# Rinoahu/SwiftOrtho

Measured on AMD Instinct MI355X. Metric: M query-aa/s scanned all-vs-all, higher is better.
Workload: dtype u8/int16/int32 (5-bit packed residues, packed 16-bit score-only DP, int32 traced DP); 1 GPU; BASELINE config 3: 100000 synthetic proteins x 300 aa self-search, seed 11111011111, aa9, -M 120000000, -c 50000 (2 chunks), -e 1e-5, -v 500; query_aa=30007201, rows=1618760

## Files before the change

swiftortho_amd/csrc/host.h:

```cpp
#pragma once
#include "common.h"
#include "kernels.h"
#include "seedhash.h"
#include "../../include/sohit.h"

#include <algorithm>
#include <array>
#include <atomic>
#include <chrono>
#include <cmath>
#include <cstring>
#include <functional>
#include <map>
#include <malloc.h>
#include <memory>
#include <mutex>
#include <thread>
#include <unordered_map>
#include <sys/stat.h>

inline double wall() { return std::chrono::duration<double>(std::chrono::steady_clock::now().time_since_epoch()).count(); }

extern double (*volatile p_pow)(double, double);
extern double (*volatile p_log)(double);
// ... 64 lines not shown
    std::string header(i64 x) const { return data.substr(hd_beg[x], hd_len[x]); }
    std::string ident(i64 x) const {
        std::string h = header(x);
        return h.substr(0, h.find(' '));
    }
    u32 len(i64 x) const { return off[x + 1] - off[x]; }
};


struct ChunkIndex {
    u64 s2 = 0;
    i64 seq_lo = 0, seq_hi = 0;
    u32 p_lo = 0, p_hi = 0;
    u32 E = 0;
    i64 threshold = 0;
    u32 maxslen = 0;
    DevBuf<u64> entries;
    DevBuf<u32> ub, ubeg, ucnt;
    u32 U = 0;
    DevBuf<u32> hkey;
    DevBuf<u64> hval;
    int hshift = 31;
    u32 hmask = 0;
    DevBuf<u64> dir;
    bool use_dir = false;
    DevBuf<u64> dkeys;
    int d_sh_subj = -1, d_sh_diag = -1;
    struct BandEnc {
        int ba = -1, bp = -1, k = -1;
        bool multi_ok = false;
        bool multi = false;
        u32 nband = 0;
        u32 C = 0;
        DevBuf<u32> dk32, gbase;
        DevBuf<u64> btab;
        std::vector<std::pair<u32, u32>> spans;
        u64 used = 0;
        bool stale = false;
        u64 ref_gen = 0;
        i64 seq_lo = -1, seq_hi = -1;
    };
    std::vector<std::unique_ptr<BandEnc>> encs;
    u64 enc_clock = 0;
    bool ordered = false;
    DevBuf<u32> row_of_slot;
    struct RangeTab {
        int ba = -1, bp = -1, k = -1, wb = -1;
// ... 39 lines not shown
    DevBuf<int> d_bittab;
    u8 smap[256];
    signed char b62c[SCLS_N * SCLS_N];
    static const int BITTAB_N = 1 << 16;
    SeqSet ref, qry;
    std::string ref_path;
    long long ref_fsize = -1, ref_mtime_ns = -1;
    bool ref_loaded = false, qry_loaded = false, index_built = false;
    u64 ref_gen = 0;
    struct BandPlan { i64 lo, hi; int bp; bool multi_ok; int k; u64 nband; };
    std::vector<BandPlan> band_plans;
    i64 r_lo = -1, r_hi = -1;
    std::vector<std::unique_ptr<ChunkIndex>> chunks;
    std::vector<std::unique_ptr<ChunkIndex>> spare_chunks;
    std::vector<std::string> masked;
    i64 masked_lo = 0;
    std::vector<std::vector<u32>> last_cands;
    std::vector<std::array<int64_t, 8>> last_p2;
    u64 qry_gen = 0;
    i64 last_q_lo = 0;
    so_counters cnt;
    DevBuf<u32> d_scan_tmp, d_tmp32a, d_tmp32b;
    DevBuf<u64> d_stats;
    DevBuf<u32> d_small;
    DevBuf<u32> ix_bkt, ix_bkt2, ix_flags, ix_ridx, ix_plan, ix_tk;
    DevBuf<u64> ix_ent, ix_tv;
    DevBuf<u8> d_pcls;
    DevBuf<u8> d_sort_tmp;
    hipEvent_t ev0 = nullptr, ev1 = nullptr;
    hipStream_t st_rows = nullptr;
    hipEvent_t ev_rows = nullptr, ev_rows_done = nullptr;
    hipEvent_t ev_part[EMIT_PARTS_MAX] = {nullptr};
    hipStream_t st_side = nullptr;
    hipEvent_t ev_side_go = nullptr, ev_korder = nullptr;
    hipStream_t st_ug = nullptr;
    hipEvent_t ev_ug_go = nullptr, ev_ug_done = nullptr;
    hipEvent_t ev_bnd_go = nullptr, ev_bnd_done = nullptr;
    bool rows_in_flight = false;
    bool count_tab_now = false;
    size_t max_hits_per_pass = (size_t)1 << 30;
    u32 max_batch = 131072;
    DevBuf<u8> d_segtab, d_symmap, d_upmap, d_segmask;
    bool seg_on_device = false;
    bool q_present[256];
    void* pinned = nullptr;
    size_t pinned_cap = 0;
// ... 418 lines not shown
```

swiftortho_amd/csrc/host_index.hip:

```cpp
#include "host.h"


i64 chunk_threshold(so_ctx* c, const u32* d_counts , u64 s1, u64 s2, u64 nn) {
    const double N = (double)(nn + 1);
    const double mu = (double)s1 / N;
    long double lm = (long double)mu;
    long double ss = (long double)s2 - 2.0L * lm * (long double)s1 + (long double)nn * lm * lm;
    if (ss < 0) ss = 0;
    long double T = lm + 2.0L * sqrtl(ss / (long double)N);
    long double fl = floorl(T);
    long double margin = ((long double)nn * 8e-16L + 1e-11L) * (T + 1.0L);
    const bool forced = tune().exact_threshold;
    if (!forced && T - fl > margin && (fl + 1.0L) - T > margin) return (i64)fl;
    std::vector<u32> counts((size_t)nn);
    if (nn) HIP_CHECK(hipMemcpyAsync(counts.data(), d_counts, (size_t)nn * sizeof(u32), hipMemcpyDeviceToHost, c->st));
    HIP_CHECK(hipStreamSynchronize(c->st));
    i64 Nn = 1;
    double m = 0.;
    for (u32 v : counts)
        if (v > 0) m += (double)v, Nn += 1;
    m /= (double)Nn;
    double sd = 0.;
    for (u32 v : counts)
        if (v > 0) sd += p_pow((double)v - m, 2);
// ... 95 lines not shown
            dlap("alloc entries / grouping scratch");
            ixsort_finish(c->ix_bkt.p, c->ix_ent.p, nslots, (u32)NC, c->ix_plan.p, c->ix_tk.p, c->ix_tv.p, c->ix_bkt2.p, ch->entries.p, c->st);
            dlap("pair grouping");
            c->ix_flags.ensure((size_t)E + 4), c->ix_ridx.ensure((size_t)E + 4);
            c->d_scan_tmp.ensure(scan_u32_temp_elems((size_t)E + 1) + 8);
            launch_run_heads(c->ix_bkt2.p, E, c->ix_flags.p, c->st);
            const u32 U = d2h_u32(c, scan_u32(c->ix_flags.p, c->ix_ridx.p, E, false, c->d_scan_tmp.p, c->st));
            ch->U = U;
            ch->ub.ensure((size_t)U + 4), ch->ubeg.ensure((size_t)U + 4), ch->ucnt.ensure((size_t)U + 4);
            launch_run_list(c->ix_bkt2.p, c->ix_flags.p, c->ix_ridx.p, E, U, ch->ub.p, ch->ubeg.p, ch->ucnt.p, c->st);
            dlap("run heads / list");
            launch_index_stats(ch->ucnt.p, U, c->d_stats.p, c->st);
            u64* stats = (u64*)small_host(c);
            u32* last_lo_h = (u32*)(stats + 4);
            HIP_CHECK(hipMemcpyAsync(stats, c->d_stats.p, 4 * sizeof(u64), hipMemcpyDeviceToHost, c->st));
            HIP_CHECK(hipMemcpyAsync(last_lo_h, ch->ubeg.p + (U - 1), sizeof(u32), hipMemcpyDeviceToHost, c->st));
            HIP_CHECK(hipStreamSynchronize(c->st));
            s2 = stats[1];
            const u32 last_lo = *last_lo_h;
            dlap("stats");
            if (ch->use_dir) {
                const size_t nd = (size_t)NC / 32 + 2;
                ch->dir.ensure(nd);
                HIP_CHECK(hipMemsetAsync(ch->dir.p, 0, nd * sizeof(u64), c->st));
                launch_dir_build(ch->ub.p, U, ch->dir.p, c->st);
            } else {
                u32 cap = 1024;
                int lg = 10;
                while (cap < 2 * U) cap <<= 1, ++lg;
                ch->hkey.ensure(cap), ch->hval.ensure(cap);
                ch->hshift = 32 - lg, ch->hmask = cap - 1;
                HIP_CHECK(hipMemsetAsync(ch->hkey.p, 0xFF, (size_t)cap * sizeof(u32), c->st));
                launch_htab_insert(ch->ub.p, ch->ubeg.p, U, ch->hkey.p, ch->hval.p, ch->hshift, ch->hmask, c->st);
            }
            launch_index_fixlast(ch->entries.p, last_lo, E, c->st);
        } else if (ch->use_dir) {
            const size_t nd = (size_t)NC / 32 + 2;
            ch->dir.ensure(nd);
            ch->ubeg.ensure(4);
            HIP_CHECK(hipMemsetAsync(ch->dir.p, 0, nd * sizeof(u64), c->st));
        } else {
            ch->hkey.ensure(1024), ch->hval.ensure(1024);
            ch->hshift = 22, ch->hmask = 1023;
            HIP_CHECK(hipMemsetAsync(ch->hkey.p, 0xFF, 1024 * sizeof(u32), c->st));
        }
        dlap("directory + fixlast");
        ch->threshold = chunk_threshold(c, ch->ucnt.p, (u64)E, s2, (u64)ch->U);
        ch->s2 = s2;
        HIP_CHECK(hipStreamSynchronize(c->st));
        c->cnt.index_entries += ch->E;
        c->chunks.push_back(std::move(ch));
    }
    c->spare_chunks.clear();
    c->cnt.n_chunks = (i64)c->chunks.size();
    c->index_built = true;
    c->cnt.index_ms += (wall() - t0) * 1e3;
}


bool host_window_bucket(const so_ctx* c, const u8* seq, u32 len, u32 pos, int a, int s, u32* bucket) {
    const int k = c->cfg.klen[s];
    if ((u64)pos + (u64)k > (u64)len) return false;
    const u32 care = c->cfg.care[s];
// ... 116 lines not shown
                    }
                    const int before = (int)std::count(seen.begin(), seen.end(), e);
                    if (before >= nt) {
                        bad = true;
                        return;
                    }
                    seen.push_back(e);
                    ent[i] = e | ((u64)tags[nt - 1 - before] << 24);
                }
            });
            if (bad) throw SoError("so_load_index: " + name + ".idx does not match the loaded reference under these seeds (a slot's window does not hash to its bucket)");
        }
        ch->entries.ensure((size_t)E + 4);
        ch->ub.ensure((size_t)U + 4), ch->ubeg.ensure((size_t)U + 4), ch->ucnt.ensure((size_t)U + 4);
        if (E) HIP_CHECK(hipMemcpyAsync(ch->entries.p, ent.data(), (size_t)E * sizeof(u64), hipMemcpyHostToDevice, c->st));
        if (U) {
            HIP_CHECK(hipMemcpyAsync(ch->ub.p, ub.data(), (size_t)U * sizeof(u32), hipMemcpyHostToDevice, c->st));
            HIP_CHECK(hipMemcpyAsync(ch->ucnt.p, ucnt.data(), (size_t)U * sizeof(u32), hipMemcpyHostToDevice, c->st));
        }
        HIP_CHECK(hipMemcpyAsync(ch->ubeg.p, ubeg.data(), ((size_t)U + 1) * sizeof(u32), hipMemcpyHostToDevice, c->st));
        if (ch->use_dir) {
            const size_t nd = (size_t)NC / 32 + 2;
            ch->dir.ensure(nd);
            HIP_CHECK(hipMemsetAsync(ch->dir.p, 0, nd * sizeof(u64), c->st));
            if (U) launch_dir_build(ch->ub.p, U, ch->dir.p, c->st);
        } else {
            u32 cap = 1024;
            int lg = 10;
            while (cap < 2 * U) cap <<= 1, ++lg;
            ch->hkey.ensure(cap), ch->hval.ensure(cap);
            ch->hshift = 32 - lg, ch->hmask = cap - 1;
            HIP_CHECK(hipMemsetAsync(ch->hkey.p, 0xFF, (size_t)cap * sizeof(u32), c->st));
            if (U) launch_htab_insert(ch->ub.p, ch->ubeg.p, U, ch->hkey.p, ch->hval.p, ch->hshift, ch->hmask, c->st);
        }
        HIP_CHECK(hipStreamSynchronize(c->st));
        c->cnt.index_entries += ch->E;
        c->chunks.push_back(std::move(ch));
    }
    c->cnt.n_chunks = (i64)c->chunks.size();
    c->index_built = true;
    c->cnt.index_ms += (wall() - t0) * 1e3;
}


void band_plan(so_ctx* c, ChunkIndex& ch, int bp, bool multi_ok, int* k_out, u64* nband_out) {
    for (const auto& pl : c->band_plans)
        if (pl.lo == ch.seq_lo && pl.hi == ch.seq_hi && pl.bp == bp && pl.multi_ok == multi_ok) {
            *k_out = pl.k, *nband_out = pl.nband;
// ... 147 lines not shown
```

swiftortho_amd/csrc/host_seed.hip:

```cpp
#include "host.h"

static void defer_long_class(so_ctx* c, Batch& b, u32 q_long) {
    b.korder_async = q_long < b.nq && b.cls_sorted && b.qcls[q_long] != b.qcls[0];
    if (!b.korder_async) return;
    b.q_defer = q_long;
    while (b.q_defer > 0 && b.qcls[b.q_defer - 1] == b.qcls[q_long]) --b.q_defer;
    HIP_CHECK(hipEventRecord(c->ev_side_go, c->st));
    HIP_CHECK(hipStreamWaitEvent(c->st_side, c->ev_side_go, 0));
}

void order_queries(so_ctx* c, Batch& b) {
    const u32 q_long = b.ksc_long;
    const size_t nres = b.h_off[b.nq];
    if (q_long < b.nq) b.gx.ensure(nres + 4), b.gL.ensure(nres + 4), b.gR.ensure(nres + 4);
    defer_long_class(c, b, q_long);
    launch_ksc_order(b.dev.d_scls.p, b.dev.d_off.p, b.nq, q_long, c->cfg.mink, c->d_b62c.p, b.gx.p, b.gL.p, b.gR.p, b.korder.p, c->st,
                     b.korder_async ? c->st_side : c->st);
    if (b.korder_async) HIP_CHECK(hipEventRecord(c->ev_korder, c->st_side));
    b.korder_ready = true;
}

void order_open_queries(so_ctx* c, Batch& b, const unsigned long long* qh) {
    u32 q_long = b.nq;
    for (u32 q = b.ksc_long; q < b.nq && q_long == b.nq; ++q)
// ... 153 lines not shown
    HIP_CHECK(hipMemcpyAsync(v, c->d_small.p + SM_STASH0, 2 * sizeof(u32), hipMemcpyDeviceToHost, c->st));
    HIP_CHECK(hipStreamSynchronize(c->st));
    a = v[0], b = v[1];
}

void ensure_sort_tmp(so_ctx* c, size_t bytes) { c->d_sort_tmp.ensure(bytes + 256); }

const unsigned long long* chunk_qhits(so_ctx* c, Batch& b, int ci) {
    ChunkIndex& ch = *c->chunks[ci];
    const int AS = c->cfg.A * c->cfg.S;
    const u32 Ppad = b.dev.Ppad, NC = (u32)c->nc;
    if (b.bnd_ci == ci) {
        HIP_CHECK(hipStreamWaitEvent(c->st, c->ev_bnd_done, 0));
        std::swap(b.sbeg.p, b.sbeg2.p), std::swap(b.sbeg.cap, b.sbeg2.cap);
        std::swap(b.scnt.p, b.scnt2.p), std::swap(b.scnt.cap, b.scnt2.cap);
        std::swap(b.pcnt.p, b.pcnt2.p), std::swap(b.pcnt.cap, b.pcnt2.cap);
    } else {
        if (b.bnd_ci >= 0) HIP_CHECK(hipStreamWaitEvent(c->st, c->ev_bnd_done, 0));
        ProfTimer pt(c, &c->cnt.bounds_ms, &c->cnt.bounds_launches);
        launch_bounds(b.qbucket.p, Ppad, AS, ch.hkey.p, ch.hval.p, ch.hshift, ch.hmask, ch.use_dir ? ch.dir.p : nullptr, ch.ubeg.p, NC, ch.E, b.sbeg.p,
                      b.scnt.p, b.pcnt.p, c->st);
        pt.stop();
        if (c->profile) c->cnt.bounds_bytes += (i64)8 * AS * (i64)b.h_off[b.nq];
    }
    b.bnd_ci = -1;
    if (tune().bounds_ahead && !c->profile) {
        int nx = ci + 1;
        while (nx < (int)c->chunks.size() && (c->chunks[nx]->seq_hi == c->chunks[nx]->seq_lo || c->chunks[nx]->E == 0)) ++nx;
        if (nx < (int)c->chunks.size()) {
            ChunkIndex& cn = *c->chunks[nx];
            const size_t T = (size_t)AS * Ppad;
            b.sbeg2.ensure(T), b.scnt2.ensure(T), b.pcnt2.ensure(Ppad);
            HIP_CHECK(hipEventRecord(c->ev_bnd_go, c->st));
            HIP_CHECK(hipStreamWaitEvent(c->st_side, c->ev_bnd_go, 0));
            launch_bounds(b.qbucket.p, Ppad, AS, cn.hkey.p, cn.hval.p, cn.hshift, cn.hmask, cn.use_dir ? cn.dir.p : nullptr, cn.ubeg.p, NC, cn.E, b.sbeg2.p, b.scnt2.p,
                          b.pcnt2.p, c->st_side);
            HIP_CHECK(hipEventRecord(c->ev_bnd_done, c->st_side));
            b.bnd_ci = nx;
        }
    }
    HIP_CHECK(hipMemsetAsync(b.mark.p, 0, Ppad, c->st));
    i64 threshold = ch.threshold;
    if (c->thr >= 1 || threshold == 0) threshold = c->thr;
    b.qhits.ensure((size_t)b.nq + 2);
    if (c->h_qhits_cap < (size_t)b.nq + 1) {
        if (c->h_qhits) (void)hipHostFree(c->h_qhits);
// ... 637 lines not shown
```

swiftortho_amd/csrc/k_index.hip:

```cpp
#include "common.h"
#include "kernels.h"
#include "seedhash.h"

__global__ __launch_bounds__(TILE_POS) void k_index_windows_sparse(const u32* __restrict__ words, const u32* __restrict__ pseq, const u32* __restrict__ off, u32 p_lo,
                                                                   u32 p_hi, u32 Ppad, u32 seq_lo, SeedCfg cfg, HashLut lut, u32 step, u32* __restrict__ bkt,
                                                                   u64* __restrict__ ent) {
    __shared__ u8 s_cls[TILE_POS + MAX_SEEDLEN];
    const u32 p0 = p_lo + blockIdx.x * TILE_POS;
    stage_classes(words, p0, Ppad, s_cls);
    __syncthreads();
    const u32 p = p0 + threadIdx.x;
    if (p >= p_hi) return;
    const u32 AS = (u32)(cfg.A * cfg.S);
    const size_t base = (size_t)(p - p_lo) * AS;
    bool live = s_cls[threadIdx.x] < HCLS_SEP;
    u32 j = 0, pos = 0;
    if (live) {
        j = pseq[p];
        pos = p - (off[j] + j);
        if (step > 1 && (pos % step) != 0) live = false;
    }
    u32 bucket[MAX_PATTERNS];
    for (int a = 0; a < cfg.A; ++a) {
        const u32 mask = live ? hash_position(s_cls + threadIdx.x, cfg, lut.v[a], bucket) : 0u;
// ... 23 lines not shown
}

__global__ __launch_bounds__(256) void k_run_counts(const u32* __restrict__ ubeg, u32 U, u32* __restrict__ cnt) {
    const u32 k = blockIdx.x * 256u + threadIdx.x;
    if (k < U) cnt[k] = ubeg[k + 1] - ubeg[k];
}

__device__ __forceinline__ u32 htab_hash(u32 b, int hshift) { return (b * 2654435761u) >> hshift; }

__global__ __launch_bounds__(256) void k_htab_insert(const u32* __restrict__ ub, const u32* __restrict__ ubeg, u32 U, u32* __restrict__ hkey,
                                                     u64* __restrict__ hval, int hshift, u32 hmask) {
    const u32 k = blockIdx.x * 256u + threadIdx.x;
    if (k >= U) return;
    const u32 b = ub[k];
    u32 h = htab_hash(b, hshift);
    for (;;) {
        const u32 old = atomicCAS(&hkey[h], HTAB_EMPTY, b);
        if (old == HTAB_EMPTY) break;
        h = (h + 1u) & hmask;
    }
    hval[h] = (u64)ubeg[k] | ((u64)(ubeg[k + 1] - ubeg[k]) << 32);
}

__global__ __launch_bounds__(256) void k_dir_build(const u32* __restrict__ ub, u32 U, u32* __restrict__ dir32) {
    const u32 k = blockIdx.x * 256u + threadIdx.x;
    if (k >= U) return;
    const u32 b = ub[k], w = b >> 5;
    if (k != 0 && (ub[k - 1] >> 5) == w) return;
    u32 bits = 1u << (b & 31u);
    for (u32 j = k + 1; j < U; ++j) {
        const u32 bj = ub[j];
        if ((bj >> 5) != w) break;
        bits |= 1u << (bj & 31u);
    }
    *reinterpret_cast<uint2*>(dir32 + 2 * (size_t)w) = make_uint2(bits, k);
}

__global__ __launch_bounds__(256) void k_index_stats(const u32* __restrict__ counts, u32 NC, u64* __restrict__ stats ) {
    u64 s1 = 0, s2 = 0;
    u32 nn = 0;
    u32 mbp1 = 0;
    const size_t stride = (size_t)gridDim.x * 256 * 4;
    for (size_t i0 = ((size_t)blockIdx.x * 256 + threadIdx.x) * 4; i0 < NC; i0 += 4 * stride) {
        uint4 v[4];
#pragma unroll
        for (int u = 0; u < 4; ++u) {
            const size_t i = i0 + u * stride;
            v[u] = make_uint4(0, 0, 0, 0);
            if (i + 3 < NC) {
                v[u] = *reinterpret_cast<const uint4*>(counts + i);
            } else if (i < NC) {
                v[u].x = counts[i];
                if (i + 1 < NC) v[u].y = counts[i + 1];
                if (i + 2 < NC) v[u].z = counts[i + 2];
            }
        }
#pragma unroll
        for (int u = 0; u < 4; ++u) {
// ... 112 lines not shown
    hipLaunchKernelGGL(k_encode_band32, dim3((E + 255) / 256), dim3(256), 0, st, entries, E, ba, gbase, roff, dk32);
}

void launch_encode_delta(const u64* entries, u32 E, int sh_subj, int sh_diag, u32 maxslen, u64* dkeys, hipStream_t st) {
    if (!E) return;
    hipLaunchKernelGGL(k_encode_delta, dim3((E + 255) / 256), dim3(256), 0, st, entries, E, sh_subj, sh_diag, maxslen, dkeys);
}

void launch_index_windows_sparse(const u32* words, const u32* pseq, const u32* off, u32 p_lo, u32 p_hi, u32 Ppad, u32 seq_lo, const SeedCfg& cfg, const HashLut& lut, u32 step,
                                 u32* bkt, u64* ent, hipStream_t st) {
    if (p_hi <= p_lo) return;
    const u32 nb = (p_hi - p_lo + TILE_POS - 1) / TILE_POS;
    hipLaunchKernelGGL(k_index_windows_sparse, dim3(nb), dim3(TILE_POS), 0, st, words, pseq, off, p_lo, p_hi, Ppad, seq_lo, cfg, lut, step, bkt, ent);
}

void launch_run_heads(const u32* bkt, u32 E, u32* flags, hipStream_t st) {
    if (E) hipLaunchKernelGGL(k_run_heads, dim3((E + 255) / 256), dim3(256), 0, st, bkt, E, flags);
}
void launch_run_list(const u32* bkt, const u32* flags, const u32* ridx, u32 E, u32 U, u32* ub, u32* ubeg, u32* cnt, hipStream_t st) {
    if (!E) return;
    hipLaunchKernelGGL(k_run_list, dim3((E + 255) / 256), dim3(256), 0, st, bkt, flags, ridx, E, U, ub, ubeg);
    hipLaunchKernelGGL(k_run_counts, dim3((U + 255) / 256), dim3(256), 0, st, ubeg, U, cnt);
}
void launch_dir_build(const u32* ub, u32 U, u64* dir, hipStream_t st) {
    if (U) hipLaunchKernelGGL(k_dir_build, dim3((U + 255) / 256), dim3(256), 0, st, ub, U, reinterpret_cast<u32*>(dir));
}

void launch_htab_insert(const u32* ub, const u32* ubeg, u32 U, u32* hkey, u64* hval, int hshift, u32 hmask, hipStream_t st) {
    if (U) hipLaunchKernelGGL(k_htab_insert, dim3((U + 255) / 256), dim3(256), 0, st, ub, ubeg, U, hkey, hval, hshift, hmask);
}

void launch_index_stats(const u32* counts, u32 NC, u64* stats_buf, hipStream_t st) {
    u32 nb = (u32)std::min<size_t>(INDEX_STATS_BLOCKS, ((size_t)NC / 4 + 255) / 256 + 1);
    hipLaunchKernelGGL(k_index_stats, dim3(nb), dim3(256), 0, st, counts, NC, stats_buf + 4);
    hipLaunchKernelGGL(k_index_stats_final, dim3(1), dim3(256), 0, st, stats_buf + 4, nb, stats_buf);
}

void launch_index_fixlast(u64* entries, u32 lo, u32 E, hipStream_t st) {
    if (E == 0) return;
    hipLaunchKernelGGL(k_index_fixlast, dim3(1), dim3(256), 0, st, entries, lo, E);
}
```

swiftortho_amd/csrc/k_seed.hip:

```cpp
#include "common.h"
#include "kernels.h"
#include "refsort.h"
#include "seedhash.h"

__global__ __launch_bounds__(TILE_POS) void k_qhash(const u32* __restrict__ words, u32 Ppad, SeedCfg cfg, HashLut lut,
                                                    u32* __restrict__ qbucket) {
    __shared__ u8 s_cls[TILE_POS + MAX_SEEDLEN];
    const u32 p0 = blockIdx.x * TILE_POS;
    stage_classes(words, p0, Ppad, s_cls);
    __syncthreads();
    const u32 p = p0 + threadIdx.x;
    if (p >= Ppad) return;
    u32 bucket[MAX_PATTERNS];
    const bool dead = s_cls[threadIdx.x] >= HCLS_SEP;
    for (int a = 0; a < cfg.A; ++a) {
        u32 mask = dead ? 0u : hash_position(s_cls + threadIdx.x, cfg, lut.v[a], bucket);
        for (int s = 0; s < cfg.S; ++s) qbucket[(size_t)(a * cfg.S + s) * Ppad + p] = ((mask >> s) & 1u) ? bucket[s] : 0xFFFFFFFFu;
    }
}

template <bool DIR>
__global__ __launch_bounds__(256) void k_bounds(const u32* __restrict__ qbucket, u32 Ppad, int AS, const u32* __restrict__ hkey,
                                                const u64* __restrict__ hval, int hshift, u32 hmask, const uint2* __restrict__ dir,
                                                const u32* __restrict__ ubeg, u32 NC, u32 E, u32* __restrict__ sbeg,
                                                u32* __restrict__ scnt, u32* __restrict__ pcnt) {
    const u32 p = blockIdx.x * 256u + threadIdx.x;
    if (p >= Ppad) return;
    const i64 L = (i64)E - 1;
    u32 tot = 0;
    for (int as = 0; as < AS; ++as) {
        const size_t t = (size_t)p * AS + as;
        const u32 b = qbucket[(size_t)as * Ppad + p];
        u32 beg = 0, cnt = 0;
        if (b != 0xFFFFFFFFu && b + 1u < NC) {
            if (DIR) {
                const uint2 d = dir[b >> 5];
                const u32 bit = b & 31u;
                if ((d.x >> bit) & 1u) {
                    const u32 k = d.y + (u32)__popc(d.x & ((1u << bit) - 1u));
                    const i64 st = (i64)ubeg[k];
                    i64 ed = (i64)ubeg[k + 1];
                    ed = ed < L ? ed : L;
                    if (ed > st) beg = (u32)st, cnt = (u32)(ed - st);
                }
            } else {
                u32 h = (b * 2654435761u) >> hshift;
                for (;;) {
                    const u32 k = hkey[h];
                    if (k == b) {
                        const u64 v = hval[h];
                        const i64 st = (i64)(u32)v;
                        i64 ed = st + (i64)(u32)(v >> 32);
                        ed = ed < L ? ed : L;
                        if (ed > st) beg = (u32)st, cnt = (u32)(ed - st);
                        break;
                    }
                    if (k == HTAB_EMPTY) break;
                    h = (h + 1u) & hmask;
                }
            }
        }
        sbeg[t] = beg;
        scnt[t] = cnt;
        tot += cnt;
    }
    pcnt[p] = tot;
}

#define LDS_SORT_MAX 4096
#define KSC_BIAS (1 << 18)

template <int CAP, int LO>
__global__ __launch_bounds__(64) void k_ksc_order_lds(const u8* __restrict__ q_scls, const u32* __restrict__ qoff, u32 nq, int mink,
                                                      const signed char* __restrict__ b62c, u32* __restrict__ korder,
                                                      const u32* __restrict__ list ,
                                                      u8* __restrict__ have) {
    __shared__ signed char s_self[SCLS_N];
    constexpr int LEAFCAP = CAP <= 512 ? 128 : CAP <= 1024 ? 256 : WQS_LEAF;
    __shared__ u32 s_x[CAP];
    __shared__ u16 s_L[CAP], s_R[CAP];
    __shared__ int s_leaf[2 * LEAFCAP];
    if (threadIdx.x < SCLS_N) s_self[threadIdx.x] = b62c[threadIdx.x * SCLS_N + threadIdx.x];
    __syncthreads();
    const u32 q = list ? list[blockIdx.x] : blockIdx.x;
    if (list && have[q]) return;
    const u32 base = qoff[q];
    const int ql = (int)(qoff[q + 1] - base);
    const int nk = ql - mink + 1;
    if (nk <= LO || nk > CAP) return;
// ... 264 lines not shown
        return;
    }
    u32 carry = 0;
#pragma unroll 1
    for (int it = 0; it < LW_ITERS; ++it) {
        const u32 hl = it * 64 + lane, h = lo + hl;
        const u32 inc = wave_scan_max((u32)s_owner[hl]);
        const u32 a = max(inc, carry);
        carry = max(carry, (u32)__builtin_amdgcn_readlane((int)inc, 63));
        if (h >= H) continue;
        const u32 base = a < LW_SEEDS ? s_base[a] : cs_base[k0 + a];
        const u64 kb = a < LW_SEEDS ? s_kb[a] : cs_kbase[k0 + a];
        const ENT d = dkeys[base + h];
        keys[h] = Addend<ENT>::offset0(d, kl) ? lookup_offset0_key(Addend<ENT>::subj(d, kl), Addend<ENT>::tag(d, kl), kb, roff, kl, maxslen)
                                              : kb + Addend<ENT>::expand(d, kl);
    }
}

void launch_qhash(const u32* words, u32 Ppad, const SeedCfg& cfg, const HashLut& lut, u32* qbucket, hipStream_t st) {
    if (!Ppad) return;
    hipLaunchKernelGGL(k_qhash, dim3((Ppad + TILE_POS - 1) / TILE_POS), dim3(TILE_POS), 0, st, words, Ppad, cfg, lut, qbucket);
}

void launch_bounds(const u32* qbucket, u32 Ppad, int AS, const u32* hkey, const u64* hval, int hshift, u32 hmask, const u64* dir, const u32* ubeg,
                   u32 NC, u32 E, u32* sbeg, u32* scnt, u32* pcnt, hipStream_t st) {
    if (!Ppad) return;
    if (dir) hipLaunchKernelGGL(k_bounds<true>, dim3((Ppad + 255) / 256), dim3(256), 0, st, qbucket, Ppad, AS, hkey, hval, hshift, hmask,
                                reinterpret_cast<const uint2*>(dir), ubeg, NC, E, sbeg, scnt, pcnt);
    else hipLaunchKernelGGL(k_bounds<false>, dim3((Ppad + 255) / 256), dim3(256), 0, st, qbucket, Ppad, AS, hkey, hval, hshift, hmask,
                            (const uint2*)nullptr, ubeg, NC, E, sbeg, scnt, pcnt);
}

void launch_ksc_order(const u8* q_scls, const u32* qoff, u32 nq, u32 q_long , int mink,
                      const signed char* b62c, u64* gx, u32* gL, u32* gR , u32* korder, hipStream_t st,
                      hipStream_t st_long ) {
    if (!nq) return;
    hipLaunchKernelGGL((k_ksc_order_lds<512, 0>), dim3(nq), dim3(64), 0, st, q_scls, qoff, nq, mink, b62c, korder, nullptr, nullptr);
    hipLaunchKernelGGL((k_ksc_order_lds<1024, 512>), dim3(nq), dim3(64), 0, st, q_scls, qoff, nq, mink, b62c, korder, nullptr, nullptr);
    hipLaunchKernelGGL((k_ksc_order_lds<LDS_SORT_MAX, 1024>), dim3(nq), dim3(64), 0, st, q_scls, qoff, nq, mink, b62c, korder, nullptr, nullptr);
    if (q_long < nq)
        hipLaunchKernelGGL(k_ksc_order_g, dim3(nq - q_long), dim3(64), 0, st_long, q_scls, qoff, q_long, nq, mink, b62c, gx, gL, gR, korder, nullptr, nullptr);
}
void launch_ksc_order_list(const u8* q_scls, const u32* qoff, u32 nq, const u32* list, u32 nlist, u8* have, u32 q_long, int mink, const signed char* b62c,
                           u64* gx, u32* gL, u32* gR, u32* korder, hipStream_t st, hipStream_t st_long) {
    if (!nlist) return;
    hipLaunchKernelGGL((k_ksc_order_lds<512, 0>), dim3(nlist), dim3(64), 0, st, q_scls, qoff, nq, mink, b62c, korder, list, have);
    hipLaunchKernelGGL((k_ksc_order_lds<1024, 512>), dim3(nlist), dim3(64), 0, st, q_scls, qoff, nq, mink, b62c, korder, list, have);
    hipLaunchKernelGGL((k_ksc_order_lds<LDS_SORT_MAX, 1024>), dim3(nlist), dim3(64), 0, st, q_scls, qoff, nq, mink, b62c, korder, list, have);
    if (q_long < nq)
        hipLaunchKernelGGL(k_ksc_order_g, dim3(nlist), dim3(64), 0, st_long, q_scls, qoff, q_long, nq, mink, b62c, gx, gL, gR, korder, list, have);
}
int ksc_lds_max() { return LDS_SORT_MAX; }

// ... 46 lines not shown
```

swiftortho_amd/csrc/kernels.h:

```cpp
#pragma once
#include "common.h"

struct HashLut;

size_t scan_u32_temp_elems(size_t n);
size_t effscan_temp_elems(size_t n);
const u32* effscan(const u8* mark, const u32* scnt, size_t n, u32* hoff, u32* cidx, u32* temp, hipStream_t st);
const u32* scan_u32(const u32* in, u32* out, size_t n, bool inclusive, u32* temp, hipStream_t st);
void fill_u32(u32* p, size_t n, u32 v, hipStream_t st);
const u32* number_by_first_appearance(const int* cx, const int* cy, u32 nr, u32 n_codes, u32* first, u32* flag, u32* rank,
                                      u32* scan_tmp, int* X, int* Y, int* gene_code, hipStream_t st);
template <class K>
const u32* key_runs(const K* key, u32 n, u32* head, u32* rid, u32* scan_tmp, hipStream_t st);
void run_starts(const u32* head, const u32* rid, u32 n, const u32* d_nruns, u32* start, hipStream_t st);

size_t sort_keys_u64_temp_bytes(size_t n, int bits);
void sort_keys_u64(void* temp, size_t temp_bytes, const u64* in, u64* out, size_t n, int begin_bit, int end_bit, hipStream_t st);
void launch_query_segments(const u32* hoff, const u32* qoff, u32 qa, u32 qb, int AS, u32 H, u32* seg, hipStream_t st);
size_t sort_keys_u64_seg_temp_bytes(size_t n, u32 nseg, int begin_bit, int end_bit);
void sort_keys_u64_seg(void* temp, size_t temp_bytes, const u64* in, u64* out, size_t n, u32 nseg, const u32* seg, int begin_bit,
                       int end_bit, hipStream_t st);
void sort_keys_u64_seg2(void* temp, size_t temp_bytes, const u64* in, u64* out, size_t n, u32 nseg, const u32* seg_begin, const u32* seg_end, int begin_bit,
                        int end_bit, hipStream_t st);
void launch_stride_gather(const u32* src, u32 stride, u32 n, u32* dst, hipStream_t st);
// ... 10 lines not shown
void ixsort_finish(u32* kin, u64* vin, u32 n, u32 NC, const u32* plan, u32* tk, u64* tv, u32* kout, u64* vout, hipStream_t st);
void launch_index_windows_sparse(const u32* words, const u32* pseq, const u32* off, u32 p_lo, u32 p_hi, u32 Ppad, u32 seq_lo, const SeedCfg& cfg, const HashLut& lut, u32 step,
                                 u32* bkt, u64* ent, hipStream_t st);

void launch_layout(const u8* res, const u32* off, u32 nseq, u32 P, u32 Ppad, const u8* hmap, u32* pseq, u8* pcls, u32* words,
                   hipStream_t st);
#define PCLS_PAD 48
struct AlnSide { const u8 *res, *scls, *scls4, *pcls, *pcls4; const u32 *off, *bound; };
struct AlnSeqs { AlnSide q, r; const signed char* b62 ; };
void launch_pad_cls(const u8* scls, const u32* off, u32 nseq, u8* out , u8* out4,
                    hipStream_t st);
#define SCLS_PAD_FRONT 16
#define SCLS_PAD_BACK 64
void launch_scls(const u8* res, size_t n, const u8* smap, u8* scls, u8* scls4 , hipStream_t st);
void launch_seq_bound(const u8* scls, const u32* off, u32 nseq, const signed char* b62c_host, u32* bound, hipStream_t st);
void launch_seg(const u8* raw, const u32* src_off, u32 q_lo, const u32* qid, u32 nq, const u32* dst_off, const u8* symmap, const u8* upmap,
                const void* tab, u8* mk, u8* out, u32 max_len, u32 q_mid, u32 q_long, hipStream_t st, hipStream_t st_long);
void launch_gather_seqs(const u8* raw, const u32* src_off, u32 q_lo, const u32* qid, u32 nq, const u32* dst_off, u8* out, hipStream_t st);
void launch_copy_range(const u8* src, u8* dst, size_t n, hipStream_t st);

#define HTAB_EMPTY 0xFFFFFFFFu
void launch_run_heads(const u32* bkt, u32 E, u32* flags, hipStream_t st);
void launch_run_list(const u32* bkt, const u32* flags, const u32* ridx, u32 E, u32 U, u32* ub, u32* ubeg, u32* cnt, hipStream_t st);
void launch_dir_build(const u32* ub, u32 U, u64* dir , hipStream_t st);
void launch_htab_insert(const u32* ub, const u32* ubeg, u32 U, u32* hkey, u64* hval, int hshift, u32 hmask, hipStream_t st);
#define INDEX_STATS_BLOCKS 2048
void launch_index_stats(const u32* counts, u32 NC, u64* stats_buf , hipStream_t st);
void launch_encode_band32(const u64* entries, u32 E, int ba, const u32* gbase , const u32* roff , u32* dk32, hipStream_t st);
void launch_encode_delta(const u64* entries, u32 E, int sh_subj, int sh_diag, u32 maxslen, u64* dkeys, hipStream_t st);
void launch_index_fixlast(u64* entries, u32 lo, u32 E, hipStream_t st);

void launch_qhash(const u32* words, u32 Ppad, const SeedCfg& cfg, const HashLut& lut, u32* qbucket, hipStream_t st);
void launch_bounds(const u32* qbucket, u32 Ppad, int AS, const u32* hkey, const u64* hval, int hshift, u32 hmask, const u64* dir ,
                   const u32* ubeg, u32 NC, u32 E, u32* sbeg, u32* scnt, u32* pcnt, hipStream_t st);
void launch_ksc_order(const u8* q_scls, const u32* qoff, u32 nq, u32 q_long , int mink,
                      const signed char* b62c, u64* gx, u32* gL, u32* gR , u32* korder, hipStream_t st,
                      hipStream_t st_long );
int ksc_lds_max();
void launch_ksc_order_list(const u8* q_scls, const u32* qoff, u32 nq, const u32* list, u32 nlist, u8* have, u32 q_long, int mink, const signed char* b62c,
                           u64* gx, u32* gL, u32* gR, u32* korder, hipStream_t st, hipStream_t st_long);
void launch_cap_all(const u32* qoff, u32 nq, int mink, const u32* pcnt, i64 threshold, u8* mark, unsigned long long* qhits, unsigned long long* over,
                    u32* open_list, hipStream_t st);
void launch_cap(const u32* korder, const u32* qoff, u32 q0, u32 nq , int mink, const u32* pcnt, i64 threshold, u8* mark,
                unsigned long long* qhits, const u32* list, u32 nlist, hipStream_t st);
void launch_effcnt(const u8* mark, const u32* scnt, int AS, u32 p_lo, u32 p_hi, u32* eff, u32* nz, hipStream_t st);
void launch_compact_seeds(const u8* mark, const u32* scnt, const u32* hoff, const u32* cidx, const u32* sbeg, const u32* q_pseq, const u32* qoff,
                          u32 p_lo, u32 p_hi, int AS, const KeyLayout& kl, u32* cs_hoff, u32* cs_beg, u64* cs_kbase, hipStream_t st);
u32 lookup_num_blocks(u32 H);
void launch_lookup_blockfirst(const u32* cs_hoff, u32 K, u32 H, u32* wave_first, hipStream_t st);
void launch_lookup(const u32* cs_hoff, const u32* cs_base, const u64* cs_kbase, const u32* wave_first, u32 K, u32 H,
                   const void* dkeys , bool compact, const u32* roff, const KeyLayout& kl, u32 maxslen,
                   u64* keys, hipStream_t st);

void launch_group_list(const u32* flags, const u32* gidx, u32 H, u32* ghead, hipStream_t st);
u32 ungap_shard_cap(u32 H);
void launch_ungap(const u64* keys, u32 H, const KeyLayout& kl, const KeyLayout& klr, const void* btab, bool gallop, bool ft_walk, const u8* q_scls, const u32* qoff,
                  const u8* r_scls, const u32* roff, const signed char* b62g, u32* shard_cnt, u32 shard_cap, u64* p_qs, u64* p_sd,
// ... 154 lines not shown
```

swiftortho_amd/csrc/tune.h:

```cpp
#pragma once
#include <cstdlib>

#define SOHIT_TUNE_TABLE(X)                                                                                                                                     \
                                                                                                                              \
    X(B, ug1, "SOHIT_UG1", 1, "bucketed passes: singleton groups to k_ungap1 (0: everything to k_ungap)")                                                     \
    X(B, ug1_chain, "SOHIT_UG1_CHAIN", 1, "... and the groups of two and more hits to k_ungap2 (0: to k_ungap, which then skips the singletons)")              \
    X(B, count_steps, "SOHIT_UG_COUNT", 0, "counting instances of the extension kernels: so_counters.ungap_steps, groups_single, groups_chain")                \
    X(B, ungapq, "SOHIT_UNGAPQ", 1, "sparse passes of queries up to 512 residues: hits alone on their diagonal by k_ungapq, a wave per query (0: every hit through the sorted keys)")     \
    X(I, uq_cache, "SOHIT_UQ_CACHE", -1, "... its hit ordinals per query whose index entries stay in registers between the two walks, in steps of 64 (-1: the compiled 1024; 0: every entry read twice; tests move the boundary)") \
    X(I, uq_chains, "SOHIT_UQ_CHAINS", -1, "... what it leaves over sorted per query (k_uqsort_wave: a wave's registers, k_uqsort_wg: a workgroup's LDS) and chained by k_ungap2 from the list of group heads (0: library segmented sort + k_ungap + k_first_touch; N > 0: the largest tier holds N keys -- tests reach the in-place instance with small inputs)") \
    X(B, ug_w32, "SOHIT_UG_W32", 1, "bucketed passes hand k_ungap the buckets' 32-bit words (0: 64-bit keys; no k_ungap1 then)")                               \
                                                                                                             \
    X(B, bucket, "SOHIT_BUCKET", 1, "bucketed diagonal binning (0: every pass on the sorted path)")                                                            \
    X(I, bucket_min, "SOHIT_BUCKET_MIN", 192, "hits per bucket below which a pass takes the sorted path (0: bucketed whenever possible)")                      \
    X(I, bucket_avg, "SOHIT_BUCKET_AVG", 2560, "average bucket size the band-range width is chosen for")                                                       \
    X(I, count_tab, "SOHIT_COUNT_TAB", 1, "bucketed passes: hits per (tile, range) from the range boundaries of the ordered index buckets when a batch brings a chunk two passes and more (0: always the counting pass over the entries; 2: always both, compared -- tests; 3: always)") \
    X(B, bucket_best, "SOHIT_BUCKET_BEST", 1, "best diagonal per subject by the per-bucket reduction (0: sort of the pass records)")                           \
    X(B, bands, "SOHIT_BANDS", 1, "diagonal bands follow the subjects' lengths (0: one band per subject)")                                                     \
    X(B, lk_wide, "SOHIT_LK_WIDE", 0, "8-byte index addends whatever the field widths")                                                                        \
    X(B, qclass, "SOHIT_QCLASS", 1, "queries of a batch in length-class order (0: file order)")                                                                \
    X(B, pass_merge, "SOHIT_PASS_MERGE", 1, "neighbouring length classes that take the sorted path anyway share one pass")                                     \
    X(B, ksc_lazy, "SOHIT_KSC_LAZY", 1, "k-mer orders computed for the queries that reach their frequency cap, when they do (a query below it keeps every window whatever the order; 0: for every query, with the batch)") \
    X(B, bounds_ahead, "SOHIT_BOUNDS_AHEAD", 1, "the next chunk's bucket bounds (k_bounds) on the side stream beside this chunk's seed stage (0: in front of its own)")     \
    X(I, segsort, "SOHIT_SEGSORT", 1, "sorted path: segmented sort of the keys inside each query (0: device-wide sort)")                                        \
// ... 13 lines not shown
    X(I, trace_var_max, "SOHIT_TRACE_VAR_MAX", -1, "tests: trace words a launch list's own-size traces may take, and the fixed-stride slabs' budget (-1: 2^31 / 2^30)") \
    X(I, emit_parts, "SOHIT_EMIT_PARTS", 4, "... and otherwise")                                                                                               \
    X(I, emit_min_rows, "SOHIT_EMIT_MIN_ROWS", 1 << 18, "rows below which the emission is one part")                                                           \
    X(P, test_oom_phase2, "SOHIT_TEST_OOM_PHASE2", 0, "tests: phase 2 of the first batch fails once with an out-of-memory error")                              \
                                                                                                                                 \
    X(I, batch, "SOHIT_BATCH", 0, "queries per device batch (0: 131072, lowered when the candidate estimate asks)")                                            \
    X(I, max_hits, "SOHIT_MAX_HITS", 0, "seed hits per pass (0: 2^30)")                                                                                        \
    X(I, poison, "SOHIT_POISON", -1, "tests: byte every fresh device allocation is filled with (-1: none)")                                                    \
    X(B, hit_cache, "SOHIT_HIT_CACHE", 1, "one released result array is kept for the next search")                                                             \
    X(P, keep_cands, "SOHIT_KEEP_CANDS", 0, "tests: keep every query's candidate list (so_query_candidates)")                                                  \
    X(P, keep_masked, "SOHIT_KEEP_MASKED", 0, "tests: keep the masked queries (so_masked_query)")                                                              \
    X(I, mcl_scratch, "SOHIT_MCL_SCRATCH", -1, "tests: u32 words of expansion / convergence scratch per range of rows (-1: 2^28)")                             \
                                                                                      \
    X(T, orth_tier, "SOHIT_ORTH_TIER", 0, "tests: every run of query rows through one tier of k_orth_run wherever that tier can take it (0 = auto: by run length)") \
                                                                                                  \
    X(T, rbh_tier, "SOHIT_RBH_TIER", 0, "tests: wave = runs of up to 64 rows through k_rbh_run_wave (what auto does), long or sort = every run through the sorted tier (0 = auto: by run length)") \
                                                                                            \
    X(T, pan_tier, "SOHIT_PAN_TIER", 0, "tests: lds = what auto does where the taxa fit the LDS of k_pan_curve, global = words, orders and counters in global memory (0 = auto: by the number of taxa)") \
                                                                                                   \
    X(I, operon_expand, "SOHIT_OPERON_EXPAND", -1, "tests: expansions per batch (-1: 2^28)")                                                                   \
                                                                                                                                           \
    X(P, exact_threshold, "SOHIT_EXACT_THRESHOLD", 0, "threshold always by the sequential fp64 replay")                                                        \
    X(I, dir_max, "SOHIT_DIR_MAX", -1, "largest -M served by the bitmap + rank directory (-1: 2^31)")                                                          \
    X(I, ixs_k, "SOHIT_IXS_K", -1, "pair grouping, second hop: slices per workgroup, a power of two up to 64 (-1: the compiled 16)")                            \
    X(I, ixs_cap, "SOHIT_IXS_CAP", -1, "pair grouping, bins: most pairs of a bin ordered in the LDS, up to 4096 (-1: 4096; 0: every bin by the counters per id; tests move the boundary)") \
                                                                                                                                          \
    X(P, debug, "SOHIT_DEBUG", 0, "per-pass lines on stderr")                                                                                                  \
    X(P, debug_index, "SOHIT_DEBUG_INDEX", 0, "wall laps of the index build on stderr")

#define ORTH_WAVE_ROWS 64
#define ORTH_LDS_ROWS 1024
#define ORTH_LDS_TAXA 512
enum { ORTH_TIER_AUTO = 0, ORTH_TIER_WAVE = 1, ORTH_TIER_LDS = 2, ORTH_TIER_SCRATCH = 3 };
static inline int orth_tier_of(const char* v) {
    switch (v[0]) {
        case 'w': case '1': return ORTH_TIER_WAVE;
        case 'l': case '2': return ORTH_TIER_LDS;
        case 's': case '3': return ORTH_TIER_SCRATCH;
        case 'g': return ORTH_TIER_SCRATCH;
        default: return ORTH_TIER_AUTO;
    }
}

#define RBH_WAVE_ROWS 64

#define PAN_LDS_BYTES 65536u
// ... 42 lines not shown
```

Before: 712.7 M query-aa/s.

## Inline bucket group sizes into the directory record to skip ubeg lookups

Each directory word grows from a bitmap plus rank to a 16-byte record. The record also holds the group's first entry offset and eight 4-bit bucket sizes where they fit. k_bounds can then compute a bucket's start and count from the record alone with a nibble prefix sum, avoiding two dependent random reads of ubeg. The trade-off is double the directory footprint, which means more cache pressure on the dir gather, plus a fallback path when sizes overflow. An optional profiling counter kernel reports how often the inline path answers.

After: 725.4 M query-aa/s (median of 6 runs). Within noise of the previous version (+1.8%).

```diff
diff --git a/swiftortho_amd/csrc/host.h b/swiftortho_amd/csrc/host.h
--- a/swiftortho_amd/csrc/host.h
+++ b/swiftortho_amd/csrc/host.h
@@ -110,7 +110,7 @@
     DevBuf<u64> hval;
     int hshift = 31;
     u32 hmask = 0;
-    DevBuf<u64> dir;
+    DevBuf<uint4> dir;
     bool use_dir = false;
     DevBuf<u64> dkeys;
     int d_sh_subj = -1, d_sh_diag = -1;
@@ -196,6 +196,7 @@
     so_counters cnt;
     DevBuf<u32> d_scan_tmp, d_tmp32a, d_tmp32b;
     DevBuf<u64> d_stats;
+    DevBuf<unsigned long long> d_dir_count;
     DevBuf<u32> d_small;
     DevBuf<u32> ix_bkt, ix_bkt2, ix_flags, ix_ridx, ix_plan, ix_tk;
     DevBuf<u64> ix_ent, ix_tv;
diff --git a/swiftortho_amd/csrc/host_index.hip b/swiftortho_amd/csrc/host_index.hip
--- a/swiftortho_amd/csrc/host_index.hip
+++ b/swiftortho_amd/csrc/host_index.hip
@@ -141,8 +141,8 @@
             if (ch->use_dir) {
                 const size_t nd = (size_t)NC / 32 + 2;
                 ch->dir.ensure(nd);
-                HIP_CHECK(hipMemsetAsync(ch->dir.p, 0, nd * sizeof(u64), c->st));
-                launch_dir_build(ch->ub.p, U, ch->dir.p, c->st);
+                HIP_CHECK(hipMemsetAsync(ch->dir.p, 0, nd * sizeof(uint4), c->st));
+                launch_dir_build(ch->ub.p, ch->ubeg.p, U, ch->dir.p, c->st);
             } else {
                 u32 cap = 1024;
                 int lg = 10;
@@ -157,7 +157,7 @@
             const size_t nd = (size_t)NC / 32 + 2;
             ch->dir.ensure(nd);
             ch->ubeg.ensure(4);
-            HIP_CHECK(hipMemsetAsync(ch->dir.p, 0, nd * sizeof(u64), c->st));
+            HIP_CHECK(hipMemsetAsync(ch->dir.p, 0, nd * sizeof(uint4), c->st));
         } else {
             ch->hkey.ensure(1024), ch->hval.ensure(1024);
             ch->hshift = 22, ch->hmask = 1023;
@@ -320,8 +320,8 @@
         if (ch->use_dir) {
             const size_t nd = (size_t)NC / 32 + 2;
             ch->dir.ensure(nd);
-            HIP_CHECK(hipMemsetAsync(ch->dir.p, 0, nd * sizeof(u64), c->st));
-            if (U) launch_dir_build(ch->ub.p, U, ch->dir.p, c->st);
+            HIP_CHECK(hipMemsetAsync(ch->dir.p, 0, nd * sizeof(uint4), c->st));
+            if (U) launch_dir_build(ch->ub.p, ch->ubeg.p, U, ch->dir.p, c->st);
         } else {
             u32 cap = 1024;
             int lg = 10;
diff --git a/swiftortho_amd/csrc/host_seed.hip b/swiftortho_amd/csrc/host_seed.hip
--- a/swiftortho_amd/csrc/host_seed.hip
+++ b/swiftortho_amd/csrc/host_seed.hip
@@ -199,6 +199,15 @@
                       b.scnt.p, b.pcnt.p, c->st);
         pt.stop();
         if (c->profile) c->cnt.bounds_bytes += (i64)8 * AS * (i64)b.h_off[b.nq];
+        if (c->profile && tune().dir_count && ch.use_dir) {
+            c->d_dir_count.ensure(4);
+            HIP_CHECK(hipMemsetAsync(c->d_dir_count.p, 0, 3 * sizeof(unsigned long long), c->st));
+            launch_bounds_count(b.qbucket.p, (size_t)AS * Ppad, ch.dir.p, NC, c->d_dir_count.p, c->st);
+            unsigned long long* v = (unsigned long long*)small_host(c);
+            HIP_CHECK(hipMemcpyAsync(v, c->d_dir_count.p, 3 * sizeof(unsigned long long), hipMemcpyDeviceToHost, c->st));
+            HIP_CHECK(hipStreamSynchronize(c->st));
+            c->tm["seed.dir_windows"] += (double)v[0], c->tm["seed.dir_occupied"] += (double)v[1], c->tm["seed.dir_inline"] += (double)v[2];
+        }
     }
     b.bnd_ci = -1;
     if (tune().bounds_ahead && !c->profile) {
diff --git a/swiftortho_amd/csrc/k_index.hip b/swiftortho_amd/csrc/k_index.hip
--- a/swiftortho_amd/csrc/k_index.hip
+++ b/swiftortho_amd/csrc/k_index.hip
@@ -69,18 +69,27 @@
     hval[h] = (u64)ubeg[k] | ((u64)(ubeg[k + 1] - ubeg[k]) << 32);
 }
 
-__global__ __launch_bounds__(256) void k_dir_build(const u32* __restrict__ ub, u32 U, u32* __restrict__ dir32) {
+__global__ __launch_bounds__(256) void k_dir_build(const u32* __restrict__ ub, const u32* __restrict__ ubeg , u32 U,
+                                                   uint4* __restrict__ dir) {
     const u32 k = blockIdx.x * 256u + threadIdx.x;
     if (k >= U) return;
     const u32 b = ub[k], w = b >> 5;
     if (k != 0 && (ub[k - 1] >> 5) == w) return;
-    u32 bits = 1u << (b & 31u);
-    for (u32 j = k + 1; j < U; ++j) {
+    u32 bits = 0, sizes = 0, n = 0;
+    bool fits = true;
+    const u32 first = ubeg[k];
+    u32 lo = first;
+    for (u32 j = k; j < U; ++j) {
         const u32 bj = ub[j];
         if ((bj >> 5) != w) break;
         bits |= 1u << (bj & 31u);
-    }
-    *reinterpret_cast<uint2*>(dir32 + 2 * (size_t)w) = make_uint2(bits, k);
+        const u32 hi = ubeg[j + 1], c = hi - lo;
+        lo = hi;
+        if (n < DIR_FIELDS && c <= DIR_FIELD_MAX) sizes |= c << (DIR_FIELD_BITS * n);
+        else fits = false;
+        ++n;
+    }
+    dir[w] = make_uint4(bits, k, first, fits ? sizes : 0u);
 }
 
 __global__ __launch_bounds__(256) void k_index_stats(const u32* __restrict__ counts, u32 NC, u64* __restrict__ stats ) {
@@ -239,8 +248,8 @@
     hipLaunchKernelGGL(k_run_list, dim3((E + 255) / 256), dim3(256), 0, st, bkt, flags, ridx, E, U, ub, ubeg);
     hipLaunchKernelGGL(k_run_counts, dim3((U + 255) / 256), dim3(256), 0, st, ubeg, U, cnt);
 }
-void launch_dir_build(const u32* ub, u32 U, u64* dir, hipStream_t st) {
-    if (U) hipLaunchKernelGGL(k_dir_build, dim3((U + 255) / 256), dim3(256), 0, st, ub, U, reinterpret_cast<u32*>(dir));
+void launch_dir_build(const u32* ub, const u32* ubeg, u32 U, uint4* dir, hipStream_t st) {
+    if (U) hipLaunchKernelGGL(k_dir_build, dim3((U + 255) / 256), dim3(256), 0, st, ub, ubeg, U, dir);
 }
 
 void launch_htab_insert(const u32* ub, const u32* ubeg, u32 U, u32* hkey, u64* hval, int hshift, u32 hmask, hipStream_t st) {
diff --git a/swiftortho_amd/csrc/k_seed.hip b/swiftortho_amd/csrc/k_seed.hip
--- a/swiftortho_amd/csrc/k_seed.hip
+++ b/swiftortho_amd/csrc/k_seed.hip
@@ -19,9 +19,14 @@
     }
 }
 
-template <bool DIR>
+__device__ __forceinline__ u32 nibble_sum(u32 w) {
+    const u32 s = (w & 0x0F0F0F0Fu) + ((w >> 4) & 0x0F0F0F0Fu);
+    return (s * 0x01010101u) >> 24;
+}
+
+template <bool DIR, bool INL>
 __global__ __launch_bounds__(256) void k_bounds(const u32* __restrict__ qbucket, u32 Ppad, int AS, const u32* __restrict__ hkey,
-                                                const u64* __restrict__ hval, int hshift, u32 hmask, const uint2* __restrict__ dir,
+                                                const u64* __restrict__ hval, int hshift, u32 hmask, const uint4* __restrict__ dir,
                                                 const u32* __restrict__ ubeg, u32 NC, u32 E, u32* __restrict__ sbeg,
                                                 u32* __restrict__ scnt, u32* __restrict__ pcnt) {
     const u32 p = blockIdx.x * 256u + threadIdx.x;
@@ -34,12 +39,26 @@
         u32 beg = 0, cnt = 0;
         if (b != 0xFFFFFFFFu && b + 1u < NC) {
             if (DIR) {
-                const uint2 d = dir[b >> 5];
+                uint4 d;
+                if (INL) {
+                    d = dir[b >> 5];
+                } else {
+                    const uint2 d2 = *reinterpret_cast<const uint2*>(dir + (b >> 5));
+                    d = make_uint4(d2.x, d2.y, 0u, 0u);
+                }
                 const u32 bit = b & 31u;
                 if ((d.x >> bit) & 1u) {
-                    const u32 k = d.y + (u32)__popc(d.x & ((1u << bit) - 1u));
-                    const i64 st = (i64)ubeg[k];
-                    i64 ed = (i64)ubeg[k + 1];
+                    const u32 j = (u32)__popc(d.x & ((1u << bit) - 1u));
+                    i64 st, ed;
+                    if (INL && d.w != 0u) {
+                        const u32 sh = DIR_FIELD_BITS * j;
+                        st = (i64)d.z + (i64)nibble_sum(d.w & ((1u << sh) - 1u));
+                        ed = st + (i64)((d.w >> sh) & DIR_FIELD_MAX);
+                    } else {
+                        const u32 k = d.y + j;
+                        st = (i64)ubeg[k];
+                        ed = (i64)ubeg[k + 1];
+                    }
                     ed = ed < L ? ed : L;
                     if (ed > st) beg = (u32)st, cnt = (u32)(ed - st);
                 }
@@ -65,6 +84,27 @@
         tot += cnt;
     }
     pcnt[p] = tot;
+}
+
+__global__ __launch_bounds__(256) void k_bounds_count(const u32* __restrict__ qbucket, size_t n, const uint4* __restrict__ dir, u32 NC,
+                                                      unsigned long long* __restrict__ out) {
+    const size_t i = (size_t)blockIdx.x * 256u + threadIdx.x;
+    u32 asked = 0, occ = 0, inl = 0;
+    if (i < n) {
+        const u32 b = qbucket[i];
+        if (b != 0xFFFFFFFFu && b + 1u < NC) {
+            const uint4 d = dir[b >> 5];
+            asked = 1;
+            occ = (d.x >> (b & 31u)) & 1u;
+            inl = occ & (d.w != 0u ? 1u : 0u);
+        }
+    }
+    const u32 a = (u32)__popcll(__ballot(asked)), o = (u32)__popcll(__ballot(occ)), w = (u32)__popcll(__ballot(inl));
+    if ((threadIdx.x & 63u) == 0 && a) {
+        atomicAdd(out + 0, (unsigned long long)a);
+        if (o) atomicAdd(out + 1, (unsigned long long)o);
+        if (w) atomicAdd(out + 2, (unsigned long long)w);
+    }
 }
 
 #define LDS_SORT_MAX 4096
@@ -375,13 +415,21 @@
     hipLaunchKernelGGL(k_qhash, dim3((Ppad + TILE_POS - 1) / TILE_POS), dim3(TILE_POS), 0, st, words, Ppad, cfg, lut, qbucket);
 }
 
-void launch_bounds(const u32* qbucket, u32 Ppad, int AS, const u32* hkey, const u64* hval, int hshift, u32 hmask, const u64* dir, const u32* ubeg,
+void launch_bounds(const u32* qbucket, u32 Ppad, int AS, const u32* hkey, const u64* hval, int hshift, u32 hmask, const uint4* dir, const u32* ubeg,
                    u32 NC, u32 E, u32* sbeg, u32* scnt, u32* pcnt, hipStream_t st) {
     if (!Ppad) return;
-    if (dir) hipLaunchKernelGGL(k_bounds<true>, dim3((Ppad + 255) / 256), dim3(256), 0, st, qbucket, Ppad, AS, hkey, hval, hshift, hmask,
-                                reinterpret_cast<const uint2*>(dir), ubeg, NC, E, sbeg, scnt, pcnt);
-    else hipLaunchKernelGGL(k_bounds<false>, dim3((Ppad + 255) / 256), dim3(256), 0, st, qbucket, Ppad, AS, hkey, hval, hshift, hmask,
-                            (const uint2*)nullptr, ubeg, NC, E, sbeg, scnt, pcnt);
+    const dim3 grid((Ppad + 255) / 256), block(256);
+    if (dir && tune().dir_inline)
+        hipLaunchKernelGGL((k_bounds<true, true>), grid, block, 0, st, qbucket, Ppad, AS, hkey, hval, hshift, hmask, dir, ubeg, NC, E, sbeg, scnt, pcnt);
+    else if (dir)
+        hipLaunchKernelGGL((k_bounds<true, false>), grid, block, 0, st, qbucket, Ppad, AS, hkey, hval, hshift, hmask, dir, ubeg, NC, E, sbeg, scnt, pcnt);
+    else
+        hipLaunchKernelGGL((k_bounds<false, false>), grid, block, 0, st, qbucket, Ppad, AS, hkey, hval, hshift, hmask, (const uint4*)nullptr, ubeg, NC, E,
+                           sbeg, scnt, pcnt);
+}
+
+void launch_bounds_count(const u32* qbucket, size_t n, const uint4* dir, u32 NC, unsigned long long* out , hipStream_t st) {
+    if (n) hipLaunchKernelGGL(k_bounds_count, dim3((unsigned)((n + 255) / 256)), dim3(256), 0, st, qbucket, n, dir, NC, out);
 }
 
 void launch_ksc_order(const u8* q_scls, const u32* qoff, u32 nq, u32 q_long , int mink,
diff --git a/swiftortho_amd/csrc/kernels.h b/swiftortho_amd/csrc/kernels.h
--- a/swiftortho_amd/csrc/kernels.h
+++ b/swiftortho_amd/csrc/kernels.h
@@ -56,7 +56,10 @@
 #define HTAB_EMPTY 0xFFFFFFFFu
 void launch_run_heads(const u32* bkt, u32 E, u32* flags, hipStream_t st);
 void launch_run_list(const u32* bkt, const u32* flags, const u32* ridx, u32 E, u32 U, u32* ub, u32* ubeg, u32* cnt, hipStream_t st);
-void launch_dir_build(const u32* ub, u32 U, u64* dir , hipStream_t st);
+#define DIR_FIELDS 8u
+#define DIR_FIELD_BITS 4u
+#define DIR_FIELD_MAX 15u
+void launch_dir_build(const u32* ub, const u32* ubeg , u32 U, uint4* dir , hipStream_t st);
 void launch_htab_insert(const u32* ub, const u32* ubeg, u32 U, u32* hkey, u64* hval, int hshift, u32 hmask, hipStream_t st);
 #define INDEX_STATS_BLOCKS 2048
 void launch_index_stats(const u32* counts, u32 NC, u64* stats_buf , hipStream_t st);
@@ -65,8 +68,9 @@
 void launch_index_fixlast(u64* entries, u32 lo, u32 E, hipStream_t st);
 
 void launch_qhash(const u32* words, u32 Ppad, const SeedCfg& cfg, const HashLut& lut, u32* qbucket, hipStream_t st);
-void launch_bounds(const u32* qbucket, u32 Ppad, int AS, const u32* hkey, const u64* hval, int hshift, u32 hmask, const u64* dir ,
+void launch_bounds(const u32* qbucket, u32 Ppad, int AS, const u32* hkey, const u64* hval, int hshift, u32 hmask, const uint4* dir ,
                    const u32* ubeg, u32 NC, u32 E, u32* sbeg, u32* scnt, u32* pcnt, hipStream_t st);
+void launch_bounds_count(const u32* qbucket, size_t n, const uint4* dir, u32 NC, unsigned long long* out , hipStream_t st);
 void launch_ksc_order(const u8* q_scls, const u32* qoff, u32 nq, u32 q_long , int mink,
                       const signed char* b62c, u64* gx, u32* gL, u32* gR , u32* korder, hipStream_t st,
                       hipStream_t st_long );
diff --git a/swiftortho_amd/csrc/tune.h b/swiftortho_amd/csrc/tune.h
--- a/swiftortho_amd/csrc/tune.h
+++ b/swiftortho_amd/csrc/tune.h
@@ -59,6 +59,8 @@
                                                                                                                                            \
     X(P, exact_threshold, "SOHIT_EXACT_THRESHOLD", 0, "threshold always by the sequential fp64 replay")                                                        \
     X(I, dir_max, "SOHIT_DIR_MAX", -1, "largest -M served by the bitmap + rank directory (-1: 2^31)")                                                          \
+    X(B, dir_inline, "SOHIT_DIR_INLINE", 1, "k_bounds takes a bucket's bounds from the directory record alone where the record holds its group's sizes (0: every group through the rank and ubeg)") \
+    X(B, dir_count, "SOHIT_DIR_COUNT", 0, "profiled searches count the windows that ask the directory, that meet an occupied bucket and that the record alone answers (timing keys seed.dir_windows / dir_occupied / dir_inline)") \
     X(I, ixs_k, "SOHIT_IXS_K", -1, "pair grouping, second hop: slices per workgroup, a power of two up to 64 (-1: the compiled 16)")                            \
     X(I, ixs_cap, "SOHIT_IXS_CAP", -1, "pair grouping, bins: most pairs of a bin ordered in the LDS, up to 4096 (-1: 4096; 0: every bin by the counters per id; tests move the boundary)") \
                                                                                                                                           \
```
